# nubomedia/NUBOMEDIA-VCA

Measured on AMD Instinct MI355X. Metric: 1080p frames/sec/node (NuboFaceDetector); achieved HBM GB/s vs peak, higher is better.
Workload: dtype i32 rect sums / f32 products / f64 stage sums (u8 pixels)

## Files before the change

### nubomedia-vca_amd/csrc/detect_job.cpp

```cpp
#include "host_state.h"
#include "host_logic.h"
#include <cstdio>
#include <cstring>
#include <algorithm>
#include <new>

using namespace nvca;

namespace nvca {

static ScaleSpec fb_make_spec(const DetectJob &j, int spitch, const FbStep &st, const ScanGrid &g)
{
    ScaleSpec sp;
    sp.table_factor = st.factor; sp.plane_off = 0; sp.pitch = spitch; sp.plane_rows = j.rq.rows + 1; sp.adaptive = 1;
    sp.out_factor = 0; sp.out_w = st.winw; sp.out_h = st.winh;
    for (int ix = g.startX; ix < g.endX; ix++) sp.xs.push_back(cv_round(ix * st.ystep));
    for (int iy = g.startY; iy < g.endY; iy++) sp.ys.push_back(cv_round(iy * st.ystep));
    return sp;
}

std::vector<SiLevel> si_levels(int ow, int oh, int cols, int rows, double sf, int minw, int minh, int maxw, int maxh, size_t cap)
{
    std::vector<SiLevel> lv;
    for (double factor = 1; lv.size() < cap; factor *= sf) {
        const int winw = cv_round(ow * factor), winh = cv_round(oh * factor);
        const int szw = cv_round(cols / factor), szh = cv_round(rows / factor);
        if (szw - ow + 1 <= 0 || szh - oh + 1 <= 0) break;
        if (winw > maxw || winh > maxh) break;
        if (winw < minw || winh < minh) continue;
        if (szw + 1 <= 1 + ow) continue;
        lv.push_back(SiLevel{factor, szw, szh, winw, winh});
    }
// ... 15 lines not shown
            PyrLevel L; L.f = sl.factor; L.szw = sl.szw; L.szh = sl.szh; L.winw = sl.winw; L.winh = sl.winh;
            L.gpitch = (int)round_up(L.szw, 64); L.gray_off = np->gray_total; L.plane_off = (int)np->plane_total;
            np->gray_total += round_up((size_t)L.gpitch * L.szh, 256);
            np->plane_total += round_up((size_t)np->P * (L.szh + 1), 64);
            np->lv.push_back(L);
        }
        std::vector<ScaleSpec> specs;
        for (const PyrLevel &L : np->lv) {
            std::unique_ptr<GeomPlan> gp(new GeomPlan());
            build_resize_tab(cols, rows, L.szw, L.szh, gp->tab);
            np->level_tabs.push_back(std::move(gp));
            ScaleSpec sp;
            sp.table_factor = 1.; sp.plane_off = L.plane_off; sp.pitch = np->P; sp.plane_rows = L.szh + 1; sp.adaptive = 0;
            sp.out_factor = L.f; sp.out_w = L.winw; sp.out_h = L.winh;
            const int ystep = L.f > 2 ? 1 : 2;
            for (int x = 0; x < L.szw - c.ow; x += ystep) sp.xs.push_back(x);
            for (int y = 0; y < L.szh - c.oh; y += ystep) sp.ys.push_back(y);
            specs.push_back(std::move(sp));
        }
        if ((rc = upload_tabs(ctx, np->level_tabs, np->d_level_tabs))) return rc;
        if (!np->lv.empty()) {
            std::string err;
            if ((rc = np->det.build_custom(ctx, c, std::move(specs), false, err))) { ctx->set_error(err); return rc; }
            if ((rc = np->det.upload(ctx))) return rc;
            std::vector<PyrLevelDev> dl(np->lv.size());
            np->pyr_ok = !ctx->sw.pyr_off;
            for (size_t li = 0; li < np->lv.size(); li++) {
                const PyrLevel &L = np->lv[li]; GeomPlan *t = np->level_tabs[li].get();
                PyrLevelDev &d = dl[li]; memset(&d, 0, sizeof(d));
                d.szw = L.szw; d.szh = L.szh; d.gpitch = L.gpitch; d.mode = t->tab.mode; d.xmax = t->tab.xmax; d.plane_off = L.plane_off;
                d.gray_off = (long long)L.gray_off;
                d.xofs = t->d_xofs.as<int>(); d.ialpha = t->d_ialpha.as<short>(); d.yofs = t->d_yofs.as<int>(); d.ibeta = t->d_ibeta.as<short>();
// ... 280 lines not shown
```

### nubomedia-vca_amd/csrc/device_records.h

```cpp
#pragma once
#include <stdint.h>
#include <stddef.h>

#if defined(__HIPCC__)
#define NVCA_HD __host__ __device__
#else
#define NVCA_HD
#endif

namespace nvca {

struct StageRec {
    int first, count; float thr;
    int flags;
    int thr_i;
    int vote_exp;
    int spec_run;
    int pad1;
};

struct ScaleRec {
    int    winw, winh;
    int    plane_off;
    int    pitch;
    int    endX, endY;
    int    eq[4];
    int    xpos_off, ypos_off;
    int    sq32;
    int    task_off;
    int    wpr;
    int    adaptive;
    double inv_area;
    double factor;
    const struct TStumpRec *trecs;
    const struct GNodeRec *grecs;
    const struct LStumpRec *lrecs;
};

struct GNodeRec {
    short dx[3][4], dy[3][4];
    float w[3];
    float thr;
// ... 30 lines not shown
static constexpr int kDeepMaxSide = 64;
static constexpr int kDeepMaxSpan = 1280;
struct BandRec { int scale, iy0, ny, first_tile, ntiles, pad0, pad1, pad2; };
static constexpr int kTileWin = 32;
static constexpr int kTileRows = 16;
static constexpr int kTileSlots = kTileWin * kTileRows;
static constexpr int kTileThreads = kTileSlots;
static constexpr int kTilesPerCu = 3;
static constexpr int kTileWavesPerSimd = (kTilesPerCu * kTileThreads / 64 + 3) / 4;
static constexpr int kTileLdsBudget = 52 * 1024;
static_assert(kTilesPerCu * kTileLdsBudget <= 160 * 1024 && kTilesPerCu * kTileThreads <= 32 * 64, "tile residency per CU");
static constexpr int kTileMaxCols = 256;
NVCA_HD inline int tile_pitch(int ncol) { return ncol | 1; }
NVCA_HD inline int tile_lds_fixed()
{
    return kTileSlots * 8 + 2 * kTileSlots * 2 + 4 * kTileWin + 128 + kTileSlots * 8;
}
NVCA_HD inline int tile_lds_bytes(int ncol, int nrow, int span_x, int span_y)
{
    return 4 * nrow * tile_pitch(ncol) + 2 * ((span_x + 3) & ~3) + 2 * ((span_y + 3) & ~3) + tile_lds_fixed();
}

static constexpr int kStripMaxWin = 512;
static constexpr int kIntegralBand = 16;

struct PreGeom {
    int sw, sh, sstride, cn;
    int w, h, gpitch;
    int spitch;
    int nbands;
    size_t src_slot, gray_slot, sum_slot, band_slot;
// ... 86 lines not shown
```

### nubomedia-vca_amd/csrc/kernels_cascade_tile.hip

```cpp
#include "launch.h"
#include "cascade_device.h"
#include <mutex>

namespace nvca {

template <class T> __device__ __forceinline__ T load_const(const T *p)
{
    static_assert(sizeof(T) % 4 == 0, "dword records only");
    typedef const __attribute__((address_space(4))) int CInt;
    CInt *q = (CInt *)p;
    T r;
    int *d = (int *)&r;
#pragma unroll
    for (int i = 0; i < (int)(sizeof(T) / 4); i++) d[i] = q[i];
    return r;
}

struct ScaleHot {
    int plane_off, pitch, eq[4], xpos_off, ypos_off, sq32, task_off, wpr, adaptive;
    double inv_area;
    const TStumpRec *trecs; const LStumpRec *lrecs;
};
__device__ __forceinline__ ScaleHot load_scale(const ScaleRec *p)
{
    typedef const __attribute__((address_space(4))) ScaleRec CScaleRec;
    CScaleRec *q = (CScaleRec *)p;
    ScaleHot h;
    h.plane_off = q->plane_off; h.pitch = q->pitch;
#pragma unroll
    for (int i = 0; i < 4; i++) h.eq[i] = q->eq[i];
    h.xpos_off = q->xpos_off; h.ypos_off = q->ypos_off; h.sq32 = q->sq32; h.task_off = q->task_off; h.wpr = q->wpr; h.adaptive = q->adaptive;
    h.inv_area = q->inv_area;
    h.trecs = q->trecs; h.lrecs = q->lrecs;
    return h;
}
struct TileScale {
    int pitch, xpos_off, ypos_off, wpr;
    const char *sum;
    double *vnf;
    const TStumpRec *trecs; const LStumpRec *lrecs;
};
__device__ __forceinline__ TileScale tile_scale(const CascadeArgs &a, const ScaleHot &h, int slot)
{
    TileScale ts;
    ts.pitch = h.pitch; ts.xpos_off = h.xpos_off; ts.ypos_off = h.ypos_off; ts.wpr = h.wpr;
    ts.sum = (const char *)(a.sum + (size_t)slot * a.sum_slot + h.plane_off);
    ts.vnf = a.vnf + ((size_t)slot * a.ntasks + h.task_off) * 64;
    ts.trecs = h.trecs; ts.lrecs = h.lrecs;
    return ts;
}


typedef int int16v __attribute__((ext_vector_type(16)));
typedef int int8v __attribute__((ext_vector_type(8)));
struct SRec { int16v a; int8v b; };
__device__ __forceinline__ SRec load_srec(const TStumpRec *p)
{
    SRec r;
    asm volatile("s_load_dwordx16 %0, %2, 0x0\n\ts_load_dwordx8 %1, %2, 0x40\n\ts_waitcnt lgkmcnt(0)"
                 : "=&s"(r.a), "=&s"(r.b) : "s"(p) : "memory");
    return r;
}
typedef __attribute__((address_space(1))) const void *gptr_t;
typedef __attribute__((address_space(3))) void *lptr_t;
typedef __attribute__((address_space(3))) const unsigned short lds_cu16;
typedef __attribute__((address_space(3))) const int lds_ci32;
#pragma clang diagnostic push
#pragma clang diagnostic ignored "-Wint-to-pointer-cast"
__device__ __forceinline__ unsigned lds_addr(const void *p) { return (unsigned)(unsigned long long)(lptr_t)p; }
__device__ __forceinline__ int lds_u16(unsigned a) { return *(lds_cu16 *)a; }
__device__ __forceinline__ int lds_sample(int r, int c)
{
    unsigned a;
    asm("v_lshl_add_u32 %0, %1, 2, %2" : "=v"(a) : "v"(r), "v"(c));
    return *(lds_ci32 *)a;
}
// ... 19 lines not shown
        const float fs = (float)s0 * w0 + (float)s1 * w1;
        v = (double)fs;
    } else {
        v = (double)((float)s0 * w0);
        v += (double)((float)s1 * w1);
        if ((f.a[15] & 255) == 3) {
            const int s2 = rs(f.a[2], f.a[5], f.a[8], f.a[11], share >> 2);
            v += (double)((float)s2 * __int_as_float(f.a[14]));
        }
    }
    if (sizeof(Sum) == sizeof(int)) return (Sum)(v >= t ? f.b[7] : f.b[6]);
    const double a0 = __hiloint2double(f.b[3], f.b[2]), a1 = __hiloint2double(f.b[5], f.b[4]);
    return (Sum)(v >= t ? a1 : a0);
}
template <bool PAIR, class Sum = double>
__device__ __forceinline__ Sum tile_stage_sum(unsigned cm, unsigned rm, double vnf, const TStumpRec *recs, int j0, int count, int step)
{
    const TStumpRec *base = recs;
    asm("" : "+v"(cm), "+v"(rm));
    Sum sum = 0;
    for (int j = j0; j < count; j += step) sum += tile_vote_s<PAIR, Sum>(cm, rm, vnf, load_srec(base + j));
    return sum;
}
__device__ __forceinline__ bool tile_stage_pass(unsigned cm, unsigned rm, double vnf, const TStumpRec *recs, const StageRec &st, bool pair)
{
    if (st.flags & 4) {
        const int sum = pair ? tile_stage_sum<true, int>(cm, rm, vnf, recs + st.first, 0, st.count, 1) : tile_stage_sum<false, int>(cm, rm, vnf, recs + st.first, 0, st.count, 1);
        return sum >= st.thr_i;
    }
    const double sum = pair ? tile_stage_sum<true>(cm, rm, vnf, recs + st.first, 0, st.count, 1) : tile_stage_sum<false>(cm, rm, vnf, recs + st.first, 0, st.count, 1);
    return !(sum < (double)st.thr);
}

struct LRec { int4 a, b, c; };
__device__ __forceinline__ LRec load_lrec(const LStumpRec *p)
{
    const int4 *q = (const int4 *)p;
    LRec r; r.a = q[0]; r.b = q[1]; r.c = q[2];
    return r;
}
__device__ __forceinline__ int lane_rect(unsigned cm, unsigned rm, unsigned xx, unsigned yy)
{
    const int c0 = lds_u16(cm + (xx & 0xffffu)), c1 = lds_u16(cm + (xx >> 16));
    const int r0 = lds_u16(rm + (yy & 0xffffu)), r1 = lds_u16(rm + (yy >> 16));
    return lds_sample(r0, c0) - lds_sample(r0, c1) - lds_sample(r1, c0) + lds_sample(r1, c1);
// ... 10 lines not shown
    else if (pair_policy && f.b.y == 1) v = (double)(p0 + p1);
    return (double)__int_as_float(v >= t ? f.c.w : f.c.z);
}

#ifdef NVCA_STAMPS
#define NVCA_STAMP(a, tile, id) do { if (threadIdx.x == 0 && blockIdx.x < 64 && (tile) < 16 && (id) < 64 && (a).dbg) { unsigned long long t__; \
    asm volatile("s_memtime %0\n\ts_waitcnt lgkmcnt(0)" : "=s"(t__) :: "memory"); (a).dbg[((size_t)blockIdx.x * 16 + (tile)) * 64 + (id)] = t__; } } while (0)
#define NVCA_STAMP_VAL(a, tile, id, v) do { if (threadIdx.x == 0 && blockIdx.x < 64 && (tile) < 16 && (id) < 64 && (a).dbg) (a).dbg[((size_t)blockIdx.x * 16 + (tile)) * 64 + (id)] = (unsigned long long)(v); } while (0)
#else
#define NVCA_STAMP(a, tile, id) do { } while (0)
#define NVCA_STAMP_VAL(a, tile, id, v) do { } while (0)
#endif

struct TileLds {
    double *acc;
    unsigned short *q0, *winx, *winy; int *qn; double *vnf_s;
    unsigned short *cmap, *rmap; int *T; int pitchT;
    int tword;
    unsigned cmA, rmA;
};
__device__ __forceinline__ TileLds carve_tile(unsigned char *lds, const TileRec &t)
{
    TileLds L;
    L.acc = (double *)lds;
    L.q0 = (unsigned short *)(lds + kTileSlots * 8);
    L.winx = L.q0 + 2 * kTileSlots; L.winy = L.winx + kTileWin;
    L.qn = (int *)(L.winy + kTileWin);
    L.vnf_s = (double *)((unsigned char *)L.qn + 128);
    L.cmap = (unsigned short *)(L.vnf_s + kTileSlots);
    L.rmap = L.cmap + ((t.span_x + 3) & ~3);
    L.T = (int *)(L.rmap + ((t.span_y + 3) & ~3));
    L.pitchT = tile_pitch(t.ncol);
    L.tword = (int)(lds_addr(L.T) >> 2);
    L.cmA = lds_addr(L.cmap); L.rmA = lds_addr(L.rmap);
    return L;
}

struct TileCoords { int mapc, mapr, wx, wy; unsigned rowy, xc[4]; };
__device__ __forceinline__ TileCoords tile_coords(const CascadeArgs &a, const TileRec &t, const TileScale &sc)
{
    const int tid = threadIdx.x, lane = tid & 63, wave = tid >> 6;
    constexpr int NW = kTileThreads / 64;
    const unsigned short *__restrict__ cl = a.tcoords + t.col_off, *__restrict__ rl = a.tcoords + t.row_off;
    TileCoords c;
    c.mapc = tid < t.ncol ? (int)cl[tid] : -1;
    c.mapr = tid < t.nrow ? (int)rl[tid] : -1;
    c.wx = tid < t.nx ? a.pos[sc.xpos_off + t.ix0 + tid] : 0;
    c.wy = (tid >= 64 && tid < 64 + t.ny) ? a.pos[sc.ypos_off + t.iy0 + tid - 64] : 0;
    const int nmine = t.nrow > wave ? (t.nrow - wave + NW - 1) / NW : 0;
    c.rowy = 0u;
    if (lane < nmine) c.rowy = rl[wave + NW * lane];
#pragma unroll
    for (int k = 0; k < 4; k++) { const int q = lane + 64 * k; c.xc[k] = cl[q < t.ncol ? q : t.ncol - 1]; }
    return c;
}
__device__ __forceinline__ void tile_commit(const TileRec &t, const TileScale &sc, const TileLds &L, const TileCoords &c)
{
    const int tid = threadIdx.x, lane = tid & 63, wave = __builtin_amdgcn_readfirstlane(tid >> 6);
    constexpr int NW = kTileThreads / 64;
    const char *__restrict__ src = sc.sum;
    const int nmine = t.nrow > wave ? (t.nrow - wave + NW - 1) / NW : 0;
    const int nk = (t.ncol + 63) >> 6;
    for (int j = 0; j < nmine; j++) {
        const unsigned rb = (unsigned)__builtin_amdgcn_readlane((int)c.rowy, j) * (unsigned)sc.pitch * 4u;
        const char *rowp = src + rb;
        int *dst = L.T + (wave + NW * j) * L.pitchT;
#pragma unroll
        for (int k = 0; k < 4; k++)
            if (k < nk && lane + 64 * k < t.ncol)
                __builtin_amdgcn_global_load_lds((gptr_t)(rowp + 4u * c.xc[k]), (lptr_t)(dst + 64 * k), 4, 0, 0);
    }
    if (tid < 3) L.qn[tid] = 0;
    if (tid < t.nx) L.winx[tid] = (unsigned short)(c.wx - t.x0);
    if (tid >= 64 && tid < 64 + t.ny) L.winy[tid - 64] = (unsigned short)(c.wy - t.y0);
    if (c.mapc >= 0) L.cmap[c.mapc - t.x0] = (unsigned short)(tid * 4);
    if (c.mapr >= 0) L.rmap[c.mapr - t.y0] = (unsigned short)(L.tword + tid * L.pitchT);
}

__device__ __forceinline__ void queue_push_wave0(bool keep, int w, unsigned short *q, int *count)
{
    if (threadIdx.x >= 64) return;
    const int lane = threadIdx.x;
    const unsigned long long km = __ballot(keep);
    if (keep) q[__popcll(km & ((1ull << lane) - 1ull))] = (unsigned short)w;
    if (lane == 0) *count = __popcll(km);
}
__device__ __forceinline__ void queue_push(bool keep, int w, unsigned short *q, int *count)
{
    const int lane = threadIdx.x & 63;
    const unsigned long long km = __ballot(keep);
    if (km) {
        int wbase = 0;
        if (lane == 0) wbase = atomicAdd(count, __popcll(km));
        wbase = __shfl(wbase, 0);
        if (keep) q[wbase + __popcll(km & ((1ull << lane) - 1ull))] = (unsigned short)w;
    }
}

static constexpr int kStatStages = 6;
static constexpr int kPairMax = 32;
static_assert(7 * kPairMax <= kTileSlots && 64 + kTileRows <= kTileThreads && kTileRows <= kTileWin,
              "a round's seven accumulator rows fit the tile's accumulators; threads 64 .. 64 + kTileRows - 1 fill winy[kTileWin]");
template <bool VNF_LDS>
__device__ __forceinline__ void tile_stages(const CascadeArgs &a, const TileRec &t, const TileScale &sc, int slot, const TileLds &L, int ti = 0, int par = 0)
{
    const int tid = threadIdx.x, lane = tid & 63;
    const int wave = __builtin_amdgcn_readfirstlane(tid >> 6);
    const int *stat_r = L.qn + 4 + par * kStatStages;
    int *stat_w = L.qn + 4 + (par ^ 1) * kStatStages;
    constexpr int NW = kTileThreads / 64;
    const TStumpRec *urecs = sc.trecs;
    const double *__restrict__ vnfp = sc.vnf + (size_t)t.iy0 * sc.wpr * 64;
    auto vnf_of = [&](int w) {
        if (VNF_LDS) return L.vnf_s[w];
        const int ix = t.ix0 + (w & 31);
        return vnfp[((size_t)(w >> 5) * sc.wpr + (ix >> 6)) * 64 + (ix & 63)];
    };
    int *acci = (int *)L.acc;
    int cur = 0;
    int cin = 0;
    const int last = a.deep_stage < a.nstages ? a.deep_stage : a.nstages;
    const int m = (last < kStatStages ? last : kStatStages) - 1;
    const bool adapt = a.stage_order && m >= 2;
    unsigned ordpack = 0x54321u;
    if (adapt) {
        const unsigned o = (unsigned)__builtin_amdgcn_readfirstlane(stat_r[0]);
        unsigned seen = 0;
        for (int q = 0; q < m; q++) seen |= 1u << ((o >> (4 * q)) & 15u);
        if (seen == (2u << m) - 2u) ordpack = o;
    }
    int kpos = 0, prev = 0; unsigned entered = 0;
    auto stage_at = [&](int kp) { return __builtin_amdgcn_readfirstlane((adapt && kp < m) ? (int)((ordpack >> (4 * kp)) & 15u) : kp + 1); };
// ... 24 lines not shown
            if (!in_prefix) {
                int lim = st.spec_run < last - s ? st.spec_run : last - s;
                if (lim > 7) lim = 7;
#pragma unroll
                for (int q = 1; q < 7; q++)
                    if (mm == q && q < lim && n * (F.v[q + 1] - F.v[0]) <= a.spec_pairs) mm = q + 1;
            }
            const int g0 = F.v[0];
            int g1 = F.v[1];
#pragma unroll
            for (int q = 2; q < 8; q++) if (mm >= q) g1 = F.v[q];
            const unsigned inv = 65535u / (unsigned)n + 1u;
            const int cc = (int)(((unsigned)lane * inv) >> 16), j = lane - cc * n;
            if (cc < G) {
                const int w = qi[j];
                const unsigned cm = L.cmA + 2 * L.winx[w & 31], rm = L.rmA + 2 * L.winy[w >> 5];
                const double vnf = vnf_of(w);
                for (int g = g0 + wave * G + cc; g < g1; g += NW * G) {
                    const LRec f = load_lrec(sc.lrecs + g);
                    const int r = (g >= F.v[1]) + (g >= F.v[2]) + (g >= F.v[3]) + (g >= F.v[4]) + (g >= F.v[5]) + (g >= F.v[6]);
                    atomicAdd(&L.acc[r * kPairMax + j], lane_vote(cm, rm, vnf, f, a.pair_policy));
                }
            }
            NVCA_STAMP(a, ti, 8 + 8 * s + 1);
            __syncthreads();
            NVCA_STAMP(a, ti, 8 + 8 * s + 2);
            bool pass = false; int w = 0;
            if (tid < n) {
                pass = true;
#pragma unroll
                for (int r = 0; r < 7; r++)
                    if (r < mm) {
// ... 10 lines not shown
        } else if (st.flags & 6) {
            const bool ints = (st.flags & 4) != 0;
            const int C = st.count;
            const int rem = n & 63, nfull = n >> 6;
            const bool rem_pair = rem > 0 && rem <= a.pair_max;
            const int Gr = rem_pair ? 64 / rem : 1;
            const int lead = (rem_pair ? nfull : (n + 63) >> 6) * C;
            const int items = lead + (rem_pair ? (C + Gr - 1) / Gr : 0), K = (items + NW - 1) / NW;
            const double vscale = ints ? __hiloint2double((1023 - st.vote_exp) << 20, 0) : 1.;
            int e = wave * K;
            const int e1 = e + K < items ? e + K : items;
            while (e < e1 && e < lead) {
                const int top = e1 < lead ? e1 : lead;
                const int wg = e / C, c0 = e - wg * C, c1 = (C - c0 < top - e) ? C : c0 + (top - e);
                const int i = wg * 64 + lane;
                if (i < n) {
                    const int w = qi[i];
                    const int xw = L.winx[w & 31], yw = L.winy[w >> 5];
                    const double vnf = vnf_of(w);
                    const unsigned cm = L.cmA + 2 * xw, rm = L.rmA + 2 * yw;
                    if (ints) {
                        const int v = pair ? tile_stage_sum<true, int>(cm, rm, vnf, urecs + st.first, c0, c1, 1) : tile_stage_sum<false, int>(cm, rm, vnf, urecs + st.first, c0, c1, 1);
                        atomicAdd(&acci[i], v);
                    } else {
                        const double v = pair ? tile_stage_sum<true, double>(cm, rm, vnf, urecs + st.first, c0, c1, 1) : tile_stage_sum<false, double>(cm, rm, vnf, urecs + st.first, c0, c1, 1);
                        atomicAdd(&L.acc[i], v);
                    }
                }
                e += c1 - c0;
            }
            if (e < e1) {
                const unsigned inv = 65535u / (unsigned)rem + 1u;
                const int cc = (int)(((unsigned)lane * inv) >> 16), j = lane - cc * rem;
                if (cc < Gr) {
                    const int i = nfull * 64 + j;
                    const int w = qi[i];
                    const unsigned cm = L.cmA + 2 * L.winx[w & 31], rm = L.rmA + 2 * L.winy[w >> 5];
                    const double vnf = vnf_of(w);
                    double sum = 0.;
                    for (int c = (e - lead) * Gr + cc; c < (e1 - lead) * Gr && c < C; c += Gr)
                        sum += lane_vote(cm, rm, vnf, load_lrec(sc.lrecs + st.first + c), a.pair_policy);
                    if (ints) atomicAdd(&acci[i], (int)(sum * vscale)); else atomicAdd(&L.acc[i], sum);
                }
            }
            NVCA_STAMP(a, ti, 8 + 8 * s + 1);
            __syncthreads();
            NVCA_STAMP(a, ti, 8 + 8 * s + 2);
            bool pass = false; int w = 0;
            if (tid < n) {
                if (ints) { const int sa = acci[tid]; acci[tid] = 0; pass = sa >= st.thr_i; }
                else { const double sa = L.acc[tid]; L.acc[tid] = 0.; pass = !(sa < (double)st.thr); }
                w = qi[tid];
            }
            if (s < kStatStages && tid == 0) stat_w[s] = adapt ? n << 16 : n;
            if (n <= 64) queue_push_wave0(pass, w, qo, &L.qn[cout]); else queue_push(pass, w, qo, &L.qn[cout]);
            NVCA_STAMP(a, ti, 8 + 8 * s + 3);
        } else {
            for (int base = 0; base < n; base += kTileThreads) {
                const int i = base + tid;
                bool pass = false; int w = 0;
                if (i < n) {
                    w = qi[i];
                    const int xw = L.winx[w & 31], yw = L.winy[w >> 5];
                    const double vnf = vnf_of(w);
                    pass = tile_stage_pass(L.cmA + 2 * xw, L.rmA + 2 * yw, vnf, urecs, st, pair);
                }
                queue_push(pass, w, qo, &L.qn[cout]);
            }
            if (tid == 0 && s < kStatStages) stat_w[s] = adapt ? n << 16 : n;
        }
        cur ^= 1; cin = cout;
        if (in_prefix) { prev = s; entered |= 1u << s; } else prev = 0;
        kpos += adv;
        if (kpos < last - 1) {
            const int sn = stage_at(kpos);
            st = load_const(a.stages + sn); F = load_const((const I8 *)(a.stage_first + sn)); TH = load_const((const F8 *)(a.stage_thr + sn));
        }
    }
    __syncthreads();
    NVCA_STAMP(a, ti, 6);
// ... 96 lines not shown
    const TileScale sc = tile_scale(a, sh, slot);
    const unsigned *__restrict__ sql = (const unsigned *)a.sqsum + (size_t)slot * 2 * a.sum_slot + sh.plane_off;
    const uint8_t *__restrict__ sqh = (const uint8_t *)((const unsigned *)a.sqsum + (size_t)slot * 2 * a.sum_slot + a.sum_slot) + sh.plane_off;
    const bool sq_lo_only = sh.sq32 != 0;
    const int ex0 = sh.eq[0] % sh.pitch, ey0 = sh.eq[0] / sh.pitch, ex1 = sh.eq[3] % sh.pitch, ey1 = sh.eq[3] / sh.pitch;
    const double inv_area = sh.inv_area;
    const bool adaptive_x = sh.adaptive != 0;
    const StageRec st0 = load_const(a.stages);
    const bool pair0 = a.pair_policy && (st0.flags & 1);
    static_assert(kTileSlots == kTileThreads, "one window per thread and tile");
    const int w = tid, ry = w >> 5, rx = w & 31;
    unsigned carry = 0;
    TileRec t = load_const(a.tiles + b.first_tile);
    TileCoords tc = tile_coords(a, t, sc);
    tile_prologue(a, carve_tile(lds, t));
    int oxw = 0, oyw = 0;
    if (ry < t.ny && rx < t.nx) { oxw = a.pos[sc.xpos_off + t.ix0 + rx]; oyw = a.pos[sc.ypos_off + t.iy0 + ry]; }
    for (int ti = 0; ti < b.ntiles; ti++) {
        __syncthreads();
        NVCA_STAMP(a, ti, 0);
        const TileLds L = carve_tile(lds, t);
        const bool active = ry < t.ny && rx < t.nx;
        int xw = oxw, yw = oyw;
        unsigned q0 = 0, q1 = 0, q2 = 0, q3 = 0, h0 = 0, h1 = 0, h2 = 0, h3 = 0;
        if (active) {
            xw -= t.x0; yw -= t.y0;
            const unsigned off = (unsigned)((t.y0 + yw) * sc.pitch + t.x0 + xw);
            const unsigned e0 = off + sh.eq[0], e1 = off + sh.eq[1], e2 = off + sh.eq[2], e3 = off + sh.eq[3];
            q0 = sql[e0]; q1 = sql[e1]; q2 = sql[e2]; q3 = sql[e3];
            if (!sq_lo_only) { h0 = sqh[e0]; h1 = sqh[e1]; h2 = sqh[e2]; h3 = sqh[e3]; }
        }
        NVCA_STAMP(a, ti, 1);
        tile_commit(t, sc, L, tc);
        if (tid < kStatStages) L.qn[4 + ((ti + 1) & 1) * kStatStages + tid] = 0;
        TileRec tn = t; TileCoords tcn = tc; int nxw = 0, nyw = 0;
        if (ti + 1 < b.ntiles) {
            tn = load_const(a.tiles + b.first_tile + ti + 1);
            tcn = tile_coords(a, tn, sc);
            if (ry < tn.ny && rx < tn.nx) { nxw = a.pos[sc.xpos_off + tn.ix0 + rx]; nyw = a.pos[sc.ypos_off + tn.iy0 + ry]; }
        }
        NVCA_STAMP(a, ti, 2);
        asm volatile("s_waitcnt vmcnt(0)" ::: "memory");
        __syncthreads();
        NVCA_STAMP(a, ti, 3);
        asm volatile("" : "+v"(h0), "+v"(h1), "+v"(h2), "+v"(h3));
        bool pass0 = false;
        if (active) {
            const int c0 = L.cmap[xw + ex0], c1 = L.cmap[xw + ex1], r0 = L.rmap[yw + ey0], r1 = L.rmap[yw + ey1];
            const int ws = lds_sample(r0, c0) - lds_sample(r0, c1) - lds_sample(r1, c0) + lds_sample(r1, c1);
            const double mean = (double)ws * inv_area;
            double vnf;
            if (sq_lo_only) vnf = (double)(unsigned)(q0 - q1 - q2 + q3);
            else vnf = (double)(((unsigned long long)h0 << 32) | q0) - (double)(((unsigned long long)h1 << 32) | q1) -
                       (double)(((unsigned long long)h2 << 32) | q2) + (double)(((unsigned long long)h3 << 32) | q3);
// ... 23 lines not shown
            unsigned nc = 0;
#pragma unroll
            for (int h = 0; h < 2; h++) {
                const unsigned Rh = h ? (unsigned)(fb >> 32) : (unsigned)fb;
                const unsigned mk = ~(Rh << (32 - t.nx));
                int ones = mk ? __clz((int)mk) : 32;
                if (ones > t.nx) ones = t.nx;
                const unsigned p = ones == t.nx ? ((unsigned)t.nx + ((carry >> h) & 1u)) & 1u : (unsigned)ones & 1u;
                nc |= p << h;
            }
            carry = (unsigned)__builtin_amdgcn_readfirstlane((int)nc);
        }
        queue_push(keep, w, L.q0, &L.qn[0]);
        NVCA_STAMP(a, ti, 5);
        tile_stages<true>(a, t, sc, slot, L, ti, ti & 1);
        t = tn; tc = tcn; oxw = nxw; oyw = nyw;
    }
}

static int grant_lds(const void *fn, int which, int bytes, int *granted)
{
    if (bytes <= *granted) return 0;
    static std::mutex mu;
    static int dev_max[2][64] = {{0}};
    std::lock_guard<std::mutex> lk(mu);
    int dev = 0; (void)hipGetDevice(&dev); dev &= 63;
    if (bytes > dev_max[which][dev]) {
        const hipError_t e = hipFuncSetAttribute(fn, hipFuncAttributeMaxDynamicSharedMemorySize, bytes);
        if (e != hipSuccess) return (int)e;
        dev_max[which][dev] = bytes;
    }
// ... 22 lines not shown
```

### nubomedia-vca_amd/csrc/plan.cpp

```cpp
#include "plan.h"
#include <cmath>
#include <cfloat>
#include <cstring>
#include <algorithm>
#include <climits>
#include <cstdlib>

namespace nvca {

static inline int cv_round(double v) { return (int)lrint(v); }
static inline int cv_floor(double v) { return (int)floor(v); }
static inline short sat_short(int v) { return (short)(v < -32768 ? -32768 : (v > 32767 ? 32767 : v)); }

void build_resize_tab(int sw, int sh, int dw, int dh, ResizeTab &t)
{
    t.sw = sw; t.sh = sh; t.dw = dw; t.dh = dh;
    t.xofs.assign(dw, 0); t.yofs.assign(dh, 0);
    t.ialpha.assign(2 * (size_t)dw, 0); t.ibeta.assign(2 * (size_t)dh, 0);
    t.xmax = dw;
    double inv_scale_x = (double)dw / sw, inv_scale_y = (double)dh / sh;
    double scale_x = 1. / inv_scale_x, scale_y = 1. / inv_scale_y;
    int iscale_x = cv_round(scale_x), iscale_y = cv_round(scale_y);
    bool is_area_fast = std::fabs(scale_x - iscale_x) < DBL_EPSILON && std::fabs(scale_y - iscale_y) < DBL_EPSILON;
    if (sw == dw && sh == dh) { t.mode = 0; return; }
// ... 206 lines not shown
bool DetectPlan::hit_valid(unsigned key) const
{
    const size_t s = key >> key_ss, iy = (key >> key_sy) & ((1u << (key_ss - key_sy)) - 1u), ix = key & ((1u << key_sy) - 1u);
    return s < specs.size() && ix < specs[s].xs.size() && iy < specs[s].ys.size();
}

nvca_rect DetectPlan::hit_rect(unsigned key) const
{
    const int s = key >> key_ss, iy = (key >> key_sy) & ((1u << (key_ss - key_sy)) - 1u), ix = key & ((1u << key_sy) - 1u);
    const ScaleSpec &sp = specs[s];
    const int x = sp.xs[ix], y = sp.ys[iy];
    if (sp.out_factor != 0) return nvca_rect{cv_round(x * sp.out_factor), cv_round(y * sp.out_factor), sp.out_w, sp.out_h};
    return nvca_rect{x, y, sp.out_w, sp.out_h};
}

int DetectPlan::build_custom(nvca_ctx *ctx, const Cascade &c, std::vector<ScaleSpec> &&in, bool allow_tiles, std::string &err)
{
    specs = std::move(in);
    const int ns = (int)c.stages.size();
    if (ctx->sw.deep_stage > 0) { deep_stage = ctx->sw.deep_stage; return build_tables(ctx, c, allow_tiles, err); }
    if (!ctx->sw.tiles || c.generic()) { deep_stage = 6; return build_tables(ctx, c, allow_tiles, err); }
    deep_stage = ns;
    int rc = build_tables(ctx, c, allow_tiles, err);
    if (rc == NVCA_OK && !generic && ctx->sw.tiles && ns > 6 && (!strips.empty() || (min_tile_side > 0 && min_tile_side < std::min(max_tile_side, 20)))) {
        deep_stage = 6;
        rc = build_tables(ctx, c, allow_tiles, err);
    }
    return rc;
}

// ... 53 lines not shown
        if (generic) {
            int mnx = 0, mxx = 0, mny = 0, mxy = 0;
            for (const GNodeRec &g : tabp->ghost)
                for (int q = 0; q < (g.flags & 255); q++)
                    for (int e = 0; e < 4; e++) { mnx = std::min<int>(mnx, g.dx[q][e]); mxx = std::max<int>(mxx, g.dx[q][e]); mny = std::min<int>(mny, g.dy[q][e]); mxy = std::max<int>(mxy, g.dy[q][e]); }
            if (!sp.xs.empty() && !sp.ys.empty() &&
                (sp.xs.front() + mnx < 0 || sp.xs.back() + mxx >= pitch || sp.ys.front() + mny < 0 || sp.ys.back() + mxy >= sp.plane_rows + 2)) {
                err = "a feature of the cascade leaves the image at this scale"; return NVCA_ERR_UNSUPPORTED;
            }
        }
        sr.plane_off = sp.plane_off; sr.pitch = pitch; sr.adaptive = sp.adaptive;
        sr.endX = (int)sp.xs.size(); sr.endY = (int)sp.ys.size();
        if (sr.endY > 8191) { err = "image too large for the task key"; return NVCA_ERR_ARG; }
        sr.xpos_off = (int)pos.size(); pos.insert(pos.end(), sp.xs.begin(), sp.xs.end());
        sr.ypos_off = (int)pos.size(); pos.insert(pos.end(), sp.ys.begin(), sp.ys.end());
        sr.task_off = (int)tasks.size();
        sr.wpr = sr.endX > 0 ? (sr.endX + 63) / 64 : 0;
        if (sr.wpr > 128) { err = "scan row too long for the task key"; return NVCA_ERR_ARG; }
        if (sr.endX > 0)
            for (int iy = 0; iy < sr.endY; iy++)
                for (int k = 0; k < sr.wpr; k++) tasks.push_back(((unsigned)s << 20) | ((unsigned)iy << 7) | (unsigned)k);
        scales.push_back(sr);
        if (sr.endX <= 0 || sr.endY <= 0) continue;
        const int *xp = &pos[sr.xpos_off], *yp = &pos[sr.ypos_off];
        int tw = 0;
        std::vector<int> offx, offy;
        const int early_last = std::min<int>(deep_stage, (int)stages.size());
        if (use_tiles && early_last > 1) {
            const int k0 = stages[0].first, k1 = stages[early_last - 1].first + stages[early_last - 1].count;
            { const auto &co = tabp->corner_offsets(k0, k1, true); offx = co.first; offy = co.second; }
// ... 117 lines not shown
    return NVCA_OK;
}

int DetectPlan::build_scale_cascade(nvca_ctx *ctx, const Cascade &c, int cols, int rows, int pitch, double scaleFactor,
                                    int minw, int minh, int maxw, int maxh, std::string &err)
{
    std::vector<double> factors;
    scale_grid(c.ow, c.oh, cols, rows, scaleFactor, minw, minh, maxw, maxh, false, factors);
    std::vector<ScaleSpec> sp;
    for (double factor : factors) {
        const double ystep = std::max(2., factor);
        ScaleSpec s;
        s.table_factor = factor; s.plane_off = 0; s.pitch = pitch; s.plane_rows = rows + 1; s.adaptive = 1;
        s.out_factor = 0; s.out_w = cv_round(c.ow * factor); s.out_h = cv_round(c.oh * factor);
        const int endX = cv_round((cols - s.out_w) / ystep), endY = cv_round((rows - s.out_h) / ystep);
        for (int ix = 0; ix < endX; ix++) s.xs.push_back(cv_round(ix * ystep));
        for (int iy = 0; iy < endY; iy++) s.ys.push_back(cv_round(iy * ystep));
        if (!s.xs.empty() && !s.ys.empty() && (s.xs.back() + s.out_w >= cols + 1 || s.ys.back() + s.out_h >= rows + 1)) {
            err = "scan grid leaves the image"; return NVCA_ERR_ARG;
        }
        sp.push_back(std::move(s));
    }
    return build_custom(ctx, c, std::move(sp), true, err);
}

const std::pair<std::vector<int>, std::vector<int>> &ScaleTable::corner_offsets(int k0, int k1, bool with_eq)
{
    const auto key = std::make_pair(with_eq ? k0 : -1 - k0, k1);
    auto it = offsets.find(key);
    if (it != offsets.end()) return it->second;
    std::vector<int> ox, oy;
    if (with_eq) { ox.push_back(ex); ox.push_back(ex + ew); oy.push_back(ey); oy.push_back(ey + eh); }
// ... 63 lines not shown
```

### nubomedia-vca_amd/csrc/plan.h

```cpp
#pragma once
#include "context.h"

namespace nvca {

void scale_grid(int ow, int oh, int cols, int rows, double scaleFactor, int minw, int minh,
                int maxw, int maxh, bool findBiggest, std::vector<double> &factors);
struct ScaleTable {
    std::vector<TStumpRec> host;
    std::vector<LStumpRec> lhost;
    DevBuf dev;
    const LStumpRec *d_lrecs = nullptr;
    std::vector<GNodeRec> ghost;
    std::vector<float> galpha;
    std::vector<int> gcls_first;
    DevBuf gdev;
    const GNodeRec *d_grecs = nullptr; const float *d_galpha = nullptr; const int *d_gcls_first = nullptr;
    int winw = 0, winh = 0, ex = 0, ey = 0, ew = 0, eh = 0;
    double inv_area = 0, factor = 0;
    int refs = 0; uint64_t last_use = 0;
    std::map<std::pair<int, int>, std::pair<std::vector<int>, std::vector<int>>> offsets;
    const std::pair<std::vector<int>, std::vector<int>> &corner_offsets(int k0, int k1, bool with_eq);
    ~ScaleTable() { dev.release(); gdev.release(); }
};
void build_scale_table(const Cascade &c, double factor, ScaleTable &t);
ScaleTable *get_scale_table(nvca_ctx *ctx, const Cascade &c, double factor);
void free_scale_tables(nvca_ctx *ctx);
void build_stage_recs(const Cascade &c, std::vector<StageRec> &out);

struct ScaleSpec {
    double table_factor;
    int plane_off, pitch;
    int plane_rows;
    std::vector<int> xs, ys;
    int adaptive;
    double out_factor;
    int out_w, out_h;
};

struct DetectPlan {
    int cols = 0, rows = 0, spitch = 0;
    int nstumps = 0;
    std::vector<ScaleRec> scales;
    std::vector<ScaleTable *> tabs;
    void release_tables();
    std::vector<StageRec> stages;
    std::vector<float> stage_thr;
    std::vector<int> stage_first;
    std::vector<StripRec> strips;
// ... 34 lines not shown
```

Measured before the change: 21190.

## Recompute window origins on device and prefetch first stump record

Window origins are no longer stored in global position tables and staged into LDS winx/winy arrays. Tile kernels now recompute them arithmetically from a per-scale start index and step using a shared rint-based helper, and the host checks that this matches its tables. This removes global loads, LDS traffic and LDS space per tile. The stage-sum loop also issues the first scalar record load before reading the queue entry, so the two latencies overlap. The cost is a double multiply and rint per window, and the approach depends on host and device rounding agreeing.

```diff
diff --git a/nubomedia-vca_amd/csrc/detect_job.cpp b/nubomedia-vca_amd/csrc/detect_job.cpp
--- a/nubomedia-vca_amd/csrc/detect_job.cpp
+++ b/nubomedia-vca_amd/csrc/detect_job.cpp
@@ -14,8 +14,7 @@
     ScaleSpec sp;
     sp.table_factor = st.factor; sp.plane_off = 0; sp.pitch = spitch; sp.plane_rows = j.rq.rows + 1; sp.adaptive = 1;
     sp.out_factor = 0; sp.out_w = st.winw; sp.out_h = st.winh;
-    for (int ix = g.startX; ix < g.endX; ix++) sp.xs.push_back(cv_round(ix * st.ystep));
-    for (int iy = g.startY; iy < g.endY; iy++) sp.ys.push_back(cv_round(iy * st.ystep));
+    sp.fill_origins(g.startX, std::max(g.endX - g.startX, 0), g.startY, std::max(g.endY - g.startY, 0), st.ystep);
     return sp;
 }
 
@@ -61,8 +60,8 @@
             sp.table_factor = 1.; sp.plane_off = L.plane_off; sp.pitch = np->P; sp.plane_rows = L.szh + 1; sp.adaptive = 0;
             sp.out_factor = L.f; sp.out_w = L.winw; sp.out_h = L.winh;
             const int ystep = L.f > 2 ? 1 : 2;
-            for (int x = 0; x < L.szw - c.ow; x += ystep) sp.xs.push_back(x);
-            for (int y = 0; y < L.szh - c.oh; y += ystep) sp.ys.push_back(y);
+            const int nx = L.szw - c.ow > 0 ? (L.szw - c.ow + ystep - 1) / ystep : 0, ny = L.szh - c.oh > 0 ? (L.szh - c.oh + ystep - 1) / ystep : 0;
+            sp.fill_origins(0, nx, 0, ny, (double)ystep);
             specs.push_back(std::move(sp));
         }
         if ((rc = upload_tabs(ctx, np->level_tabs, np->d_level_tabs))) return rc;
diff --git a/nubomedia-vca_amd/csrc/device_records.h b/nubomedia-vca_amd/csrc/device_records.h
--- a/nubomedia-vca_amd/csrc/device_records.h
+++ b/nubomedia-vca_amd/csrc/device_records.h
@@ -1,6 +1,7 @@
 #pragma once
 #include <stdint.h>
 #include <stddef.h>
+#include <math.h>
 
 #if defined(__HIPCC__)
 #define NVCA_HD __host__ __device__
@@ -9,6 +10,15 @@
 #endif
 
 namespace nvca {
+
+NVCA_HD inline int window_origin(int i0, int i, double step)
+{
+#if defined(__HIP_DEVICE_COMPILE__)
+    return (int)__builtin_rint((double)(i0 + i) * step);
+#else
+    return (int)lrint((double)(i0 + i) * step);
+#endif
+}
 
 struct StageRec {
     int first, count; float thr;
@@ -26,6 +36,8 @@
     int    endX, endY;
     int    eq[4];
     int    xpos_off, ypos_off;
+    int    pos_ix0, pos_iy0;
+    double pos_step;
     int    sq32;
     int    task_off;
     int    wpr;
@@ -86,7 +98,7 @@
 NVCA_HD inline int tile_pitch(int ncol) { return ncol | 1; }
 NVCA_HD inline int tile_lds_fixed()
 {
-    return kTileSlots * 8 + 2 * kTileSlots * 2 + 4 * kTileWin + 128 + kTileSlots * 8;
+    return kTileSlots * 8 + 2 * kTileSlots * 2 + 128 + kTileSlots * 8;
 }
 NVCA_HD inline int tile_lds_bytes(int ncol, int nrow, int span_x, int span_y)
 {
diff --git a/nubomedia-vca_amd/csrc/kernels_cascade_tile.hip b/nubomedia-vca_amd/csrc/kernels_cascade_tile.hip
--- a/nubomedia-vca_amd/csrc/kernels_cascade_tile.hip
+++ b/nubomedia-vca_amd/csrc/kernels_cascade_tile.hip
@@ -17,8 +17,8 @@
 }
 
 struct ScaleHot {
-    int plane_off, pitch, eq[4], xpos_off, ypos_off, sq32, task_off, wpr, adaptive;
-    double inv_area;
+    int plane_off, pitch, eq[4], pos_ix0, pos_iy0, sq32, task_off, wpr, adaptive;
+    double inv_area, pos_step;
     const TStumpRec *trecs; const LStumpRec *lrecs;
 };
 __device__ __forceinline__ ScaleHot load_scale(const ScaleRec *p)
@@ -29,13 +29,14 @@
     h.plane_off = q->plane_off; h.pitch = q->pitch;
 #pragma unroll
     for (int i = 0; i < 4; i++) h.eq[i] = q->eq[i];
-    h.xpos_off = q->xpos_off; h.ypos_off = q->ypos_off; h.sq32 = q->sq32; h.task_off = q->task_off; h.wpr = q->wpr; h.adaptive = q->adaptive;
-    h.inv_area = q->inv_area;
+    h.pos_ix0 = q->pos_ix0; h.pos_iy0 = q->pos_iy0; h.sq32 = q->sq32; h.task_off = q->task_off; h.wpr = q->wpr; h.adaptive = q->adaptive;
+    h.inv_area = q->inv_area; h.pos_step = q->pos_step;
     h.trecs = q->trecs; h.lrecs = q->lrecs;
     return h;
 }
 struct TileScale {
-    int pitch, xpos_off, ypos_off, wpr;
+    int pitch, wpr;
+    int pos_ix0, pos_iy0; double pos_step;
     const char *sum;
     double *vnf;
     const TStumpRec *trecs; const LStumpRec *lrecs;
@@ -43,7 +44,7 @@
 __device__ __forceinline__ TileScale tile_scale(const CascadeArgs &a, const ScaleHot &h, int slot)
 {
     TileScale ts;
-    ts.pitch = h.pitch; ts.xpos_off = h.xpos_off; ts.ypos_off = h.ypos_off; ts.wpr = h.wpr;
+    ts.pitch = h.pitch; ts.wpr = h.wpr; ts.pos_ix0 = h.pos_ix0; ts.pos_iy0 = h.pos_iy0; ts.pos_step = h.pos_step;
     ts.sum = (const char *)(a.sum + (size_t)slot * a.sum_slot + h.plane_off);
     ts.vnf = a.vnf + ((size_t)slot * a.ntasks + h.task_off) * 64;
     ts.trecs = h.trecs; ts.lrecs = h.lrecs;
@@ -60,6 +61,16 @@
     asm volatile("s_load_dwordx16 %0, %2, 0x0\n\ts_load_dwordx8 %1, %2, 0x40\n\ts_waitcnt lgkmcnt(0)"
                  : "=&s"(r.a), "=&s"(r.b) : "s"(p) : "memory");
     return r;
+}
+__device__ __forceinline__ SRec issue_srec(const TStumpRec *p)
+{
+    SRec r;
+    asm volatile("s_load_dwordx16 %0, %2, 0x0\n\ts_load_dwordx8 %1, %2, 0x40" : "=&s"(r.a), "=&s"(r.b) : "s"(p) : "memory");
+    return r;
+}
+__device__ __forceinline__ void wait_srec(SRec &r)
+{
+    asm volatile("s_waitcnt lgkmcnt(0)" : "+s"(r.a), "+s"(r.b) : : "memory");
 }
 typedef __attribute__((address_space(1))) const void *gptr_t;
 typedef __attribute__((address_space(3))) void *lptr_t;
@@ -109,21 +120,27 @@
     return (Sum)(v >= t ? a1 : a0);
 }
 template <bool PAIR, class Sum = double>
-__device__ __forceinline__ Sum tile_stage_sum(unsigned cm, unsigned rm, double vnf, const TStumpRec *recs, int j0, int count, int step)
+__device__ __forceinline__ Sum tile_stage_sum(unsigned cm, unsigned rm, double vnf, const TStumpRec *recs, SRec f, int j0, int count)
 {
     const TStumpRec *base = recs;
     asm("" : "+v"(cm), "+v"(rm));
     Sum sum = 0;
-    for (int j = j0; j < count; j += step) sum += tile_vote_s<PAIR, Sum>(cm, rm, vnf, load_srec(base + j));
+    for (int j = j0;;) {
+        sum += tile_vote_s<PAIR, Sum>(cm, rm, vnf, f);
+        if (++j >= count) break;
+        f = load_srec(base + j);
+    }
     return sum;
 }
 __device__ __forceinline__ bool tile_stage_pass(unsigned cm, unsigned rm, double vnf, const TStumpRec *recs, const StageRec &st, bool pair)
 {
+    if (st.count <= 0) return (st.flags & 4) ? 0 >= st.thr_i : !(0. < (double)st.thr);
+    const SRec f = load_srec(recs + st.first);
     if (st.flags & 4) {
-        const int sum = pair ? tile_stage_sum<true, int>(cm, rm, vnf, recs + st.first, 0, st.count, 1) : tile_stage_sum<false, int>(cm, rm, vnf, recs + st.first, 0, st.count, 1);
+        const int sum = pair ? tile_stage_sum<true, int>(cm, rm, vnf, recs + st.first, f, 0, st.count) : tile_stage_sum<false, int>(cm, rm, vnf, recs + st.first, f, 0, st.count);
         return sum >= st.thr_i;
     }
-    const double sum = pair ? tile_stage_sum<true>(cm, rm, vnf, recs + st.first, 0, st.count, 1) : tile_stage_sum<false>(cm, rm, vnf, recs + st.first, 0, st.count, 1);
+    const double sum = pair ? tile_stage_sum<true>(cm, rm, vnf, recs + st.first, f, 0, st.count) : tile_stage_sum<false>(cm, rm, vnf, recs + st.first, f, 0, st.count);
     return !(sum < (double)st.thr);
 }
 
@@ -164,7 +181,7 @@
 
 struct TileLds {
     double *acc;
-    unsigned short *q0, *winx, *winy; int *qn; double *vnf_s;
+    unsigned short *q0; int *qn; double *vnf_s;
     unsigned short *cmap, *rmap; int *T; int pitchT;
     int tword;
     unsigned cmA, rmA;
@@ -174,8 +191,7 @@
     TileLds L;
     L.acc = (double *)lds;
     L.q0 = (unsigned short *)(lds + kTileSlots * 8);
-    L.winx = L.q0 + 2 * kTileSlots; L.winy = L.winx + kTileWin;
-    L.qn = (int *)(L.winy + kTileWin);
+    L.qn = (int *)(L.q0 + 2 * kTileSlots);
     L.vnf_s = (double *)((unsigned char *)L.qn + 128);
     L.cmap = (unsigned short *)(L.vnf_s + kTileSlots);
     L.rmap = L.cmap + ((t.span_x + 3) & ~3);
@@ -186,7 +202,7 @@
     return L;
 }
 
-struct TileCoords { int mapc, mapr, wx, wy; unsigned rowy, xc[4]; };
+struct TileCoords { int mapc, mapr; unsigned rowy, xc[4]; };
 __device__ __forceinline__ TileCoords tile_coords(const CascadeArgs &a, const TileRec &t, const TileScale &sc)
 {
     const int tid = threadIdx.x, lane = tid & 63, wave = tid >> 6;
@@ -195,8 +211,6 @@
     TileCoords c;
     c.mapc = tid < t.ncol ? (int)cl[tid] : -1;
     c.mapr = tid < t.nrow ? (int)rl[tid] : -1;
-    c.wx = tid < t.nx ? a.pos[sc.xpos_off + t.ix0 + tid] : 0;
-    c.wy = (tid >= 64 && tid < 64 + t.ny) ? a.pos[sc.ypos_off + t.iy0 + tid - 64] : 0;
     const int nmine = t.nrow > wave ? (t.nrow - wave + NW - 1) / NW : 0;
     c.rowy = 0u;
     if (lane < nmine) c.rowy = rl[wave + NW * lane];
@@ -221,8 +235,6 @@
                 __builtin_amdgcn_global_load_lds((gptr_t)(rowp + 4u * c.xc[k]), (lptr_t)(dst + 64 * k), 4, 0, 0);
     }
     if (tid < 3) L.qn[tid] = 0;
-    if (tid < t.nx) L.winx[tid] = (unsigned short)(c.wx - t.x0);
-    if (tid >= 64 && tid < 64 + t.ny) L.winy[tid - 64] = (unsigned short)(c.wy - t.y0);
     if (c.mapc >= 0) L.cmap[c.mapc - t.x0] = (unsigned short)(tid * 4);
     if (c.mapr >= 0) L.rmap[c.mapr - t.y0] = (unsigned short)(L.tword + tid * L.pitchT);
 }
@@ -249,8 +261,7 @@
 
 static constexpr int kStatStages = 6;
 static constexpr int kPairMax = 32;
-static_assert(7 * kPairMax <= kTileSlots && 64 + kTileRows <= kTileThreads && kTileRows <= kTileWin,
-              "a round's seven accumulator rows fit the tile's accumulators; threads 64 .. 64 + kTileRows - 1 fill winy[kTileWin]");
+static_assert(7 * kPairMax <= kTileSlots, "a round's seven accumulator rows fit the tile's accumulators");
 template <bool VNF_LDS>
 __device__ __forceinline__ void tile_stages(const CascadeArgs &a, const TileRec &t, const TileScale &sc, int slot, const TileLds &L, int ti = 0, int par = 0)
 {
@@ -266,6 +277,10 @@
         const int ix = t.ix0 + (w & 31);
         return vnfp[((size_t)(w >> 5) * sc.wpr + (ix >> 6)) * 64 + (ix & 63)];
     };
+    const int gx0 = sc.pos_ix0 + t.ix0, gy0 = sc.pos_iy0 + t.iy0;
+    const unsigned cmB = L.cmA - 2u * (unsigned)t.x0, rmB = L.rmA - 2u * (unsigned)t.y0;
+    auto cm_of = [&](int w) { return cmB + 2u * (unsigned)window_origin(gx0, w & 31, sc.pos_step); };
+    auto rm_of = [&](int w) { return rmB + 2u * (unsigned)window_origin(gy0, w >> 5, sc.pos_step); };
     int *acci = (int *)L.acc;
     int cur = 0;
     int cin = 0;
@@ -320,8 +335,8 @@
             const int cc = (int)(((unsigned)lane * inv) >> 16), j = lane - cc * n;
             if (cc < G) {
                 const int w = qi[j];
-                const unsigned cm = L.cmA + 2 * L.winx[w & 31], rm = L.rmA + 2 * L.winy[w >> 5];
                 const double vnf = vnf_of(w);
+                const unsigned cm = cm_of(w), rm = rm_of(w);
                 for (int g = g0 + wave * G + cc; g < g1; g += NW * G) {
                     const LRec f = load_lrec(sc.lrecs + g);
                     const int r = (g >= F.v[1]) + (g >= F.v[2]) + (g >= F.v[3]) + (g >= F.v[4]) + (g >= F.v[5]) + (g >= F.v[6]);
@@ -362,16 +377,17 @@
                 const int top = e1 < lead ? e1 : lead;
                 const int wg = e / C, c0 = e - wg * C, c1 = (C - c0 < top - e) ? C : c0 + (top - e);
                 const int i = wg * 64 + lane;
+                SRec f = issue_srec(urecs + st.first + c0);
+                const int w = qi[i < n ? i : 0];
+                wait_srec(f);
                 if (i < n) {
-                    const int w = qi[i];
-                    const int xw = L.winx[w & 31], yw = L.winy[w >> 5];
                     const double vnf = vnf_of(w);
-                    const unsigned cm = L.cmA + 2 * xw, rm = L.rmA + 2 * yw;
+                    const unsigned cm = cm_of(w), rm = rm_of(w);
                     if (ints) {
-                        const int v = pair ? tile_stage_sum<true, int>(cm, rm, vnf, urecs + st.first, c0, c1, 1) : tile_stage_sum<false, int>(cm, rm, vnf, urecs + st.first, c0, c1, 1);
+                        const int v = pair ? tile_stage_sum<true, int>(cm, rm, vnf, urecs + st.first, f, c0, c1) : tile_stage_sum<false, int>(cm, rm, vnf, urecs + st.first, f, c0, c1);
                         atomicAdd(&acci[i], v);
                     } else {
-                        const double v = pair ? tile_stage_sum<true, double>(cm, rm, vnf, urecs + st.first, c0, c1, 1) : tile_stage_sum<false, double>(cm, rm, vnf, urecs + st.first, c0, c1, 1);
+                        const double v = pair ? tile_stage_sum<true, double>(cm, rm, vnf, urecs + st.first, f, c0, c1) : tile_stage_sum<false, double>(cm, rm, vnf, urecs + st.first, f, c0, c1);
                         atomicAdd(&L.acc[i], v);
                     }
                 }
@@ -383,8 +399,8 @@
                 if (cc < Gr) {
                     const int i = nfull * 64 + j;
                     const int w = qi[i];
-                    const unsigned cm = L.cmA + 2 * L.winx[w & 31], rm = L.rmA + 2 * L.winy[w >> 5];
                     const double vnf = vnf_of(w);
+                    const unsigned cm = cm_of(w), rm = rm_of(w);
                     double sum = 0.;
                     for (int c = (e - lead) * Gr + cc; c < (e1 - lead) * Gr && c < C; c += Gr)
                         sum += lane_vote(cm, rm, vnf, load_lrec(sc.lrecs + st.first + c), a.pair_policy);
@@ -409,9 +425,8 @@
                 bool pass = false; int w = 0;
                 if (i < n) {
                     w = qi[i];
-                    const int xw = L.winx[w & 31], yw = L.winy[w >> 5];
                     const double vnf = vnf_of(w);
-                    pass = tile_stage_pass(L.cmA + 2 * xw, L.rmA + 2 * yw, vnf, urecs, st, pair);
+                    pass = tile_stage_pass(cm_of(w), rm_of(w), vnf, urecs, st, pair);
                 }
                 queue_push(pass, w, qo, &L.qn[cout]);
             }
@@ -538,17 +553,15 @@
     TileRec t = load_const(a.tiles + b.first_tile);
     TileCoords tc = tile_coords(a, t, sc);
     tile_prologue(a, carve_tile(lds, t));
-    int oxw = 0, oyw = 0;
-    if (ry < t.ny && rx < t.nx) { oxw = a.pos[sc.xpos_off + t.ix0 + rx]; oyw = a.pos[sc.ypos_off + t.iy0 + ry]; }
     for (int ti = 0; ti < b.ntiles; ti++) {
         __syncthreads();
         NVCA_STAMP(a, ti, 0);
         const TileLds L = carve_tile(lds, t);
         const bool active = ry < t.ny && rx < t.nx;
-        int xw = oxw, yw = oyw;
+        int xw = 0, yw = 0;
         unsigned q0 = 0, q1 = 0, q2 = 0, q3 = 0, h0 = 0, h1 = 0, h2 = 0, h3 = 0;
         if (active) {
-            xw -= t.x0; yw -= t.y0;
+            xw = window_origin(sc.pos_ix0 + t.ix0, rx, sc.pos_step) - t.x0; yw = window_origin(sc.pos_iy0 + t.iy0, ry, sc.pos_step) - t.y0;
             const unsigned off = (unsigned)((t.y0 + yw) * sc.pitch + t.x0 + xw);
             const unsigned e0 = off + sh.eq[0], e1 = off + sh.eq[1], e2 = off + sh.eq[2], e3 = off + sh.eq[3];
             q0 = sql[e0]; q1 = sql[e1]; q2 = sql[e2]; q3 = sql[e3];
@@ -557,11 +570,10 @@
         NVCA_STAMP(a, ti, 1);
         tile_commit(t, sc, L, tc);
         if (tid < kStatStages) L.qn[4 + ((ti + 1) & 1) * kStatStages + tid] = 0;
-        TileRec tn = t; TileCoords tcn = tc; int nxw = 0, nyw = 0;
+        TileRec tn = t; TileCoords tcn = tc;
         if (ti + 1 < b.ntiles) {
             tn = load_const(a.tiles + b.first_tile + ti + 1);
             tcn = tile_coords(a, tn, sc);
-            if (ry < tn.ny && rx < tn.nx) { nxw = a.pos[sc.xpos_off + tn.ix0 + rx]; nyw = a.pos[sc.ypos_off + tn.iy0 + ry]; }
         }
         NVCA_STAMP(a, ti, 2);
         asm volatile("s_waitcnt vmcnt(0)" ::: "memory");
@@ -615,7 +627,7 @@
         queue_push(keep, w, L.q0, &L.qn[0]);
         NVCA_STAMP(a, ti, 5);
         tile_stages<true>(a, t, sc, slot, L, ti, ti & 1);
-        t = tn; tc = tcn; oxw = nxw; oyw = nyw;
+        t = tn; tc = tcn;
     }
 }
 
diff --git a/nubomedia-vca_amd/csrc/plan.cpp b/nubomedia-vca_amd/csrc/plan.cpp
--- a/nubomedia-vca_amd/csrc/plan.cpp
+++ b/nubomedia-vca_amd/csrc/plan.cpp
@@ -244,6 +244,14 @@
     return nvca_rect{x, y, sp.out_w, sp.out_h};
 }
 
+void ScaleSpec::fill_origins(int ix0, int nx, int iy0, int ny, double step)
+{
+    pos_ix0 = ix0; pos_iy0 = iy0; pos_step = step;
+    xs.clear(); ys.clear();
+    for (int i = 0; i < nx; i++) xs.push_back(window_origin(ix0, i, step));
+    for (int i = 0; i < ny; i++) ys.push_back(window_origin(iy0, i, step));
+}
+
 int DetectPlan::build_custom(nvca_ctx *ctx, const Cascade &c, std::vector<ScaleSpec> &&in, bool allow_tiles, std::string &err)
 {
     specs = std::move(in);
@@ -327,6 +335,11 @@
         if (sr.endY > 8191) { err = "image too large for the task key"; return NVCA_ERR_ARG; }
         sr.xpos_off = (int)pos.size(); pos.insert(pos.end(), sp.xs.begin(), sp.xs.end());
         sr.ypos_off = (int)pos.size(); pos.insert(pos.end(), sp.ys.begin(), sp.ys.end());
+        sr.pos_ix0 = sp.pos_ix0; sr.pos_iy0 = sp.pos_iy0; sr.pos_step = sp.pos_step;
+        for (size_t i = 0; i < sp.xs.size(); i++)
+            if (sp.xs[i] != window_origin(sp.pos_ix0, (int)i, sp.pos_step)) { err = "internal: a scan grid's columns are not window_origin() of its step"; return NVCA_ERR_INTERNAL; }
+        for (size_t i = 0; i < sp.ys.size(); i++)
+            if (sp.ys[i] != window_origin(sp.pos_iy0, (int)i, sp.pos_step)) { err = "internal: a scan grid's rows are not window_origin() of its step"; return NVCA_ERR_INTERNAL; }
         sr.task_off = (int)tasks.size();
         sr.wpr = sr.endX > 0 ? (sr.endX + 63) / 64 : 0;
         if (sr.wpr > 128) { err = "scan row too long for the task key"; return NVCA_ERR_ARG; }
@@ -474,8 +487,7 @@
         s.table_factor = factor; s.plane_off = 0; s.pitch = pitch; s.plane_rows = rows + 1; s.adaptive = 1;
         s.out_factor = 0; s.out_w = cv_round(c.ow * factor); s.out_h = cv_round(c.oh * factor);
         const int endX = cv_round((cols - s.out_w) / ystep), endY = cv_round((rows - s.out_h) / ystep);
-        for (int ix = 0; ix < endX; ix++) s.xs.push_back(cv_round(ix * ystep));
-        for (int iy = 0; iy < endY; iy++) s.ys.push_back(cv_round(iy * ystep));
+        s.fill_origins(0, endX, 0, endY, ystep);
         if (!s.xs.empty() && !s.ys.empty() && (s.xs.back() + s.out_w >= cols + 1 || s.ys.back() + s.out_h >= rows + 1)) {
             err = "scan grid leaves the image"; return NVCA_ERR_ARG;
         }
diff --git a/nubomedia-vca_amd/csrc/plan.h b/nubomedia-vca_amd/csrc/plan.h
--- a/nubomedia-vca_amd/csrc/plan.h
+++ b/nubomedia-vca_amd/csrc/plan.h
@@ -32,6 +32,9 @@
     int plane_off, pitch;
     int plane_rows;
     std::vector<int> xs, ys;
+    int pos_ix0 = 0, pos_iy0 = 0;
+    double pos_step = 0;
+    void fill_origins(int ix0, int nx, int iy0, int ny, double step);
     int adaptive;
     double out_factor;
     int out_w, out_h;
```

New measurement: 20520. 0.968x the previous value.
